# CDCgov/zoe

Measured on AMD Instinct MI355X. Metric: read-alignments/sec (150 bp vs 2 kb ref), higher is better.
Workload: dtype int16

## Files before the change

include/zoe_sw.h:

```cpp
#ifndef ZOE_SW_H
#define ZOE_SW_H

#include <stddef.h>
#include <stdint.h>

#ifdef __cplusplus
extern "C" {
#endif

typedef enum zsw_error {
    ZSW_OK = 0,
    ZSW_ERR_EMPTY_SEQUENCE = 1,
    ZSW_ERR_GAP_OPEN_OUT_OF_RANGE = 2,
    ZSW_ERR_GAP_EXTEND_OUT_OF_RANGE = 3,
    ZSW_ERR_BAD_GAP_WEIGHTS = 4,
    ZSW_ERR_INVALID_ARGUMENT = -1,
    ZSW_ERR_HIP = -2,
    ZSW_ERR_NO_DEVICE = -3,
    ZSW_ERR_UNSUPPORTED = -4,
    ZSW_ERR_NOT_CONFIGURED = -5
} zsw_error;

typedef enum zsw_status {
    ZSW_STATUS_SOME = 0,
// ... 139 lines not shown

zsw_error zsw_group_align_batch_from(zsw_group* group, const zsw_batch* reads, int from_width, int preset_bits, int invert,
                                     zsw_alignment* out_aln, uint8_t* out_status, uint8_t* out_tier, uint32_t* out_inc,
                                     uint8_t* out_op, uint64_t ciglet_cap, uint64_t* out_n_ciglets);
zsw_error zsw_group_align_3pass_batch_from(zsw_group* group, const zsw_batch* reads, int from_width, int preset_bits, int invert,
                                           zsw_alignment* out_aln, uint8_t* out_status, uint8_t* out_tier, uint32_t* out_inc,
                                           uint8_t* out_op, uint64_t ciglet_cap, uint64_t* out_n_ciglets);

zsw_error zsw_group_score_batch_from_device(zsw_group* group, const zsw_batch* shards, int from_width, int preset_bits,
                                            uint32_t* const* out_score, uint8_t* const* out_status);

zsw_error zsw_synth_reads(zsw_context* ctx, uint64_t seed, uint64_t first, uint64_t n, uint32_t len, uint8_t* out_device,
                          void* stream);
zsw_error zsw_synth_reads_ragged(zsw_context* ctx, uint64_t seed, uint64_t first, uint64_t n, uint32_t min_len,
                                 uint32_t max_len, const uint64_t* offsets_device, uint8_t* out_device, void* stream);
uint32_t zsw_synth_length(uint64_t seed, uint64_t index, uint32_t min_len, uint32_t max_len);

zsw_error zsw_selftest(zsw_context* ctx);

void zsw_synth_reference_host(uint64_t seed, uint64_t len, uint8_t* out);
void zsw_synth_reads_host(uint64_t seed, uint64_t first, uint64_t n, uint32_t len, const uint8_t* ref, uint32_t R,
                          uint8_t* out);
void zsw_synth_reads_ragged_host(uint64_t seed, uint64_t first, uint64_t n, uint32_t min_len, uint32_t max_len,
                                 const uint64_t* offsets, const uint8_t* ref, uint32_t R, uint8_t* out);

zsw_error zsw_timing_enable(zsw_context* ctx, int enable);
zsw_error zsw_timing_read(zsw_context* ctx, double* seconds, uint64_t* launches);
zsw_error zsw_timing_read_window(zsw_context* ctx, double* seconds, uint64_t* launches);

typedef enum zsw_option { ZSW_OPTION_EXACT_PRUNING = 1, ZSW_OPTION_MIN_SCORE = 2 } zsw_option;
zsw_error zsw_set_option(zsw_context* ctx, zsw_option option, int64_t value);

zsw_error zsw_min_score_counts(zsw_context* ctx, uint64_t* out );

typedef enum zsw_debug_flag {
    ZSW_DEBUG_SCORE_V1 = 1,
    ZSW_DEBUG_NO_TILES = 2,
    ZSW_DEBUG_NO_W32 = 4,
    ZSW_DEBUG_NO_WIDE = 8,
    ZSW_DEBUG_NO_SIDE_STREAMS = 16,
    ZSW_DEBUG_NO_PIPELINE = 32,
    ZSW_DEBUG_ALIGN_NO_PACKED = 64,
    ZSW_DEBUG_SCORE_PRUNE = 128,
    ZSW_DEBUG_SCORE_PRUNE_ANY_SIZE = 256,
    ZSW_DEBUG_PRUNE_STRIP = 512,
    ZSW_DEBUG_ALIGN_LONG_WARMUP = 1024,
    ZSW_DEBUG_SEED_NO_BAND = 2048,
    ZSW_DEBUG_SEED_WIDE_BAND = 4096,
    ZSW_DEBUG_NO_ROW_CHUNKS = 8192,
    ZSW_DEBUG_RANGES_EXACT_REVERSE = 16384,
    ZSW_DEBUG_ALIGN_NO_CERTIFICATE = 32768,
    ZSW_DEBUG_SEED_STRIP_FIRST_TIER = 65536,
    ZSW_DEBUG_SEED_DIAG_LANE_EVENTS = 131072,
    ZSW_DEBUG_SEED_NO_COSCHEDULE = 262144
} zsw_debug_flag;
zsw_error zsw_debug_set(zsw_context* ctx, uint32_t flags);

zsw_error zsw_debug_band_records(zsw_context* ctx, int32_t* records);

zsw_error zsw_debug_cert_records(zsw_context* ctx, int32_t* records);

zsw_error zsw_debug_strand_records(zsw_context* ctx, int32_t* records);

typedef enum zsw_launch_kind {
    ZSW_LAUNCH_V1_FAST = 0,
    ZSW_LAUNCH_V1_BIASED = 1,
    ZSW_LAUNCH_V2 = 2,
    ZSW_LAUNCH_WIDE = 3,
    ZSW_LAUNCH_V1_FAST_REV = 4,
    ZSW_LAUNCH_V1_BIASED_REV = 5,
    ZSW_LAUNCH_WIDE_REV = 6,
    ZSW_LAUNCH_TILE_V2 = 7,
    ZSW_LAUNCH_TILE_WIDE = 8,
    ZSW_LAUNCH_TILE_W32 = 9,
    ZSW_LAUNCH_EXACT32 = 10,
    ZSW_LAUNCH_EXACT32_WORKLIST = 11,
    ZSW_LAUNCH_SEED_WINDOW = 12,
    ZSW_LAUNCH_SEED_BAND = 13,
    ZSW_LAUNCH_PRUNED = 14,
    ZSW_LAUNCH_ROW_CHUNKS = 15
} zsw_launch_kind;
zsw_error zsw_debug_score_launches(zsw_context* ctx, uint32_t* records, uint32_t capacity, uint32_t* out_n);

zsw_error zsw_prune_rescored(zsw_context* ctx, uint64_t* out_reads);

#ifdef __cplusplus
}
#endif
#endif
```

zoe_amd/_lib.py:

```python
from __future__ import annotations

import ctypes as C
import os

_HERE = os.path.dirname(os.path.abspath(__file__))
LIB_PATH = os.path.join(_HERE, "libzoe_sw_hip.so")

ZSW_OK = 0
ERROR_NAMES = {
    0: "ZSW_OK",
    1: "ProfileError::EmptySequence",
    2: "ProfileError::GapOpenOutOfRange",
    3: "ProfileError::GapExtendOutOfRange",
    4: "ProfileError::BadGapWeights",
    -1: "ZSW_ERR_INVALID_ARGUMENT",
    -2: "ZSW_ERR_HIP",
    -3: "ZSW_ERR_NO_DEVICE",
    -4: "ZSW_ERR_UNSUPPORTED",
    -5: "ZSW_ERR_NOT_CONFIGURED",
}
MEM_HOST, MEM_DEVICE = 0, 1
DEBUG_SCORE_V1, DEBUG_NO_TILES, DEBUG_NO_W32, DEBUG_NO_WIDE, DEBUG_NO_SIDE_STREAMS, DEBUG_NO_PIPELINE, DEBUG_ALIGN_NO_PACKED = 1, 2, 4, 8, 16, 32, 64
DEBUG_SCORE_PRUNE, DEBUG_SCORE_PRUNE_ANY_SIZE, DEBUG_PRUNE_STRIP, DEBUG_ALIGN_LONG_WARMUP, DEBUG_SEED_NO_BAND, DEBUG_SEED_WIDE_BAND = 128, 256, 512, 1024, 2048, 4096
DEBUG_NO_ROW_CHUNKS = 8192
DEBUG_RANGES_EXACT_REVERSE = 16384
DEBUG_ALIGN_NO_CERTIFICATE = 32768
DEBUG_SEED_STRIP_FIRST_TIER = 65536
DEBUG_SEED_DIAG_LANE_EVENTS = 131072
DEBUG_SEED_NO_COSCHEDULE = 262144
(LAUNCH_V1_FAST, LAUNCH_V1_BIASED, LAUNCH_V2, LAUNCH_WIDE, LAUNCH_V1_FAST_REV, LAUNCH_V1_BIASED_REV, LAUNCH_WIDE_REV, LAUNCH_TILE_V2, LAUNCH_TILE_WIDE,
 LAUNCH_TILE_W32, LAUNCH_EXACT32, LAUNCH_EXACT32_WORKLIST, LAUNCH_SEED_WINDOW, LAUNCH_SEED_BAND, LAUNCH_PRUNED, LAUNCH_ROW_CHUNKS) = range(16)
OPTION_EXACT_PRUNING = 1
OPTION_MIN_SCORE = 2
INT_TYPES = {"i8": 0, "i16": 1, "i32": 2, "u8": 3, "u16": 4, "u32": 5}

SYMBOLS = [
    "zsw_pack4_host", "zsw_create", "zsw_destroy", "zsw_last_error_string", "zsw_device_count", "zsw_set_scoring", "zsw_set_reference",
    "zsw_score_batch", "zsw_score_batch_from", "zsw_score_ends_batch", "zsw_score_ranges_batch", "zsw_score_ranges_batch_from", "zsw_align_batch", "zsw_align_batch_from", "zsw_align_3pass_batch", "zsw_align_3pass_batch_from", "zsw_sneaky_snake_batch",
    "zsw_set_profile_sequence", "zsw_score_shared_batch", "zsw_score_shared_batch_from", "zsw_score_ends_shared_batch", "zsw_score_ranges_shared_batch",
    "zsw_score_ranges_shared_batch_from", "zsw_align_shared_batch", "zsw_align_shared_batch_from", "zsw_align_3pass_shared_batch", "zsw_align_3pass_shared_batch_from",
    "zsw_synth_reads", "zsw_synth_reads_ragged", "zsw_synth_length", "zsw_synth_reference_host", "zsw_synth_reads_host",
    "zsw_synth_reads_ragged_host", "zsw_selftest", "zsw_timing_enable", "zsw_timing_read", "zsw_timing_read_window", "zsw_debug_set", "zsw_debug_band_records", "zsw_debug_cert_records", "zsw_prune_rescored", "zsw_set_option",
    "zsw_group_create", "zsw_group_destroy", "zsw_group_size", "zsw_group_context", "zsw_group_last_error_string", "zsw_group_set_scoring",
    "zsw_group_set_reference", "zsw_group_score_batch_from", "zsw_group_score_batch_from_device", "zsw_group_align_batch_from",
    "zsw_group_align_3pass_batch_from",
    "zsw_set_complement", "zsw_score_strands_batch_from", "zsw_orient_batch", "zsw_align_3pass_strands_batch_from", "zsw_strand_counts", "zsw_debug_strand_records", "zsw_debug_score_launches",
    "zsw_min_score_counts",
]


class ZswBatch(C.Structure):
    _fields_ = [
        ("bases", C.c_void_p),
        ("offsets", C.c_void_p),
        ("fixed_len", C.c_uint32),
        ("n_reads", C.c_uint64),
        ("mem", C.c_int),
        ("encoding", C.c_int),
    ]


class ZswAlignment(C.Structure):
    _fields_ = [
        ("score", C.c_uint32),
        ("ref_start", C.c_uint32),
        ("ref_end", C.c_uint32),
        ("query_start", C.c_uint32),
        ("query_end", C.c_uint32),
        ("ref_len", C.c_uint32),
        ("query_len", C.c_uint32),
        ("n_ciglets", C.c_uint32),
        ("ciglet_offset", C.c_uint64),
    ]


class ZswError(RuntimeError):
    def __init__(self, code: int, detail: str = ""):
        self.code = code
        name = ERROR_NAMES.get(code, str(code))
        super().__init__(f"{name}{': ' + detail if detail else ''}")


# ... 85 lines not shown
```

zoe_amd/build.py:

```python
from __future__ import annotations

import os
import shutil
import subprocess
import sys

HERE = os.path.dirname(os.path.abspath(__file__))
CSRC = os.path.join(HERE, "csrc")
LIB = os.path.join(HERE, "libzoe_sw_hip.so")
SOURCES = ["zsw_capi.hip", "zsw_capi_shared.hip", "zsw_shared.hip", "zsw_score.hip", "zsw_align.hip", "zsw_align_pk8.hip", "zsw_align_pk16.hip", "zsw_align_pk32.hip", "zsw_align_pk64.hip", "zsw_group.hip", "zsw_threepass.hip", "zsw_filter.hip", "zsw_score_wide.hip", "zsw_score_w32.hip", "zsw_score_prune.hip", "zsw_score_seed.hip", "zsw_score_seed_m0.hip", "zsw_score_seed_m1.hip", "zsw_score_seed_m2.hip", "zsw_score_band.hip", "zsw_multi.hip", "zsw_strand.hip"]
HEADERS = ["zsw_internal.hpp", "zsw_align_dev.hpp", "zsw_align_pk.hpp", "zsw_align_pk_kernel.hpp", "zsw_score_v1.hpp", "zsw_score_v2.hpp", "zsw_handback.hpp", "zsw_score_prune.hpp", "zsw_seed.hpp", "zsw_seed_diag.hpp", "zsw_seed_diag_body.inc", "zsw_cert.hpp", "zsw_context.hpp", "zsw_shared.hpp", "zsw_score_seed.hpp", "zsw_score_seed_kernel.hpp", "zsw_align.hpp", "zsw_timer.hpp", "zsw_strand.hpp", "zsw_synth.h", "zsw_exports.map", os.path.join("..", "..", "include", "zoe_sw.h")]
ARCH = "gfx950"
EXTRA_FLAGS = {}


def _hipcc() -> str:
    for cand in (shutil.which("hipcc"), "/opt/rocm/bin/hipcc"):
        if cand and os.path.exists(cand):
            return cand
    raise RuntimeError("hipcc not found: the HIP extension cannot be built")


def needs_build() -> bool:
    if not os.path.exists(LIB):
        return True
    t = os.path.getmtime(LIB)
    deps = [os.path.join(CSRC, s) for s in SOURCES + HEADERS] + [os.path.abspath(__file__)]
    return any(os.path.exists(d) and os.path.getmtime(d) > t for d in deps)


def build(force: bool = False, verbose: bool = False) -> str:
    if not force and not needs_build():
        return LIB
    objs = []
    procs = []
    for s in SOURCES:
        src = os.path.join(CSRC, s)
        if not os.path.exists(src):
            continue
        obj = os.path.join(CSRC, s.replace(".hip", ".o"))
        cmd = [_hipcc(), f"--offload-arch={ARCH}", "-O3", "-std=c++17", "-fPIC", "-c", src, "-o", obj,
               "-Wall", "-Wno-unused-function", "-Wno-unused-result"] + EXTRA_FLAGS.get(s, [])
        if verbose:
            cmd.append("-Rpass-analysis=kernel-resource-usage")
        procs.append((s, subprocess.Popen(cmd, stdout=subprocess.PIPE, stderr=subprocess.STDOUT, text=True)))
        objs.append(obj)
    failed = False
    for s, p in procs:
        out, _ = p.communicate()
        if p.returncode != 0:
            failed = True
            sys.stderr.write(f"--- hipcc failed for {s}\n{out}\n")
        elif verbose or out.strip():
            sys.stderr.write(out)
    if failed:
        raise RuntimeError("hipcc compilation failed")
    cmd = [_hipcc(), f"--offload-arch={ARCH}", "-shared", "-fPIC", "-o", LIB, "-Wl,--version-script=" + os.path.join(CSRC, "zsw_exports.map")] + objs
    subprocess.run(cmd, check=True)
    return LIB


def fatbin_sha256(path: str = LIB) -> str:
    import hashlib
    import struct
# ... 36 lines not shown
```

zoe_amd/csrc/zsw_score.hip:

```cpp
#include <stdlib.h>

#include <algorithm>

#include "zsw_internal.hpp"
#include "zsw_score_v1.hpp"
#include "zsw_score_prune.hpp"
#include "zsw_score_seed.hpp"
#include "zsw_score_v2.hpp"
#include "zsw_handback.hpp"
#include "zsw_timer.hpp"

namespace zsw {

__global__ __launch_bounds__(64) void exact32_kernel(BatchDev b, const uint32_t* list, const uint32_t* list_count,
                                                     const uint8_t* ref, uint32_t ref_len, const ScoringDev* sc,
                                                     ResultRule rule, ScoreOut out, int32_t* scratch, uint32_t slots,
                                                     uint32_t scratch_len, const uint32_t* rev_ref_end,
                                                     const uint32_t* rev_query_end) {
    __shared__ uint8_t lut[256];
    __shared__ int32_t w[MAX_S * MAX_S];
    for (int i = threadIdx.x; i < 256; i += 64) lut[i] = sc->index_map[i];
    for (int i = threadIdx.x; i < MAX_S * MAX_S; i += 64) w[i] = sc->w[i];
    __syncthreads();
    const int S = sc->S;
// ... 507 lines not shown
        note_launch(launches, ZSW_LAUNCH_EXACT32, 0, 0, std::min(mode, 2));
        hipLaunchKernelGGL(exact32_kernel, dim3(exact_grid), dim3(64), 0, stream, bb, (const uint32_t*)nullptr,
                           (const uint32_t*)nullptr, d_ref, ref_len, d_sc, rule, out, ws.scratch, (uint32_t)ws.slots, ws.scratch_len, (const uint32_t*)nullptr, (const uint32_t*)nullptr);
        return hipGetLastError();
    };
    bool gtab_built = false;
    auto seed_items = [&](const BatchDev& bb, int g, int c, uint32_t longest, size_t work_off, uint32_t list_off, uint32_t* counter,
                          uint32_t band_grid_cap) -> hipError_t {
        if (!use_v2 || !ws.seed || !ws.seed_work || !ws.prune_fail_list || !(ws.debug & ZSW_DEBUG_SCORE_PRUNE) || (ws.debug & ZSW_DEBUG_PRUNE_STRIP))
            return hipErrorNotSupported;
        if (bb.n_items < SEED_MIN_READS && !(ws.debug & ZSW_DEBUG_SCORE_PRUNE_ANY_SIZE)) return hipErrorNotSupported;
        if (g == 32 || work_off + seed_workspace_bytes(bb.n_items, longest, band_grid_cap) > ws.seed_bytes) return hipErrorNotSupported;
        ScoreArgsV2 ap = a2;
        if (!build_tables_v2(h_sc, g, &ap) || !seed_applicable(*ws.seed, longest, ref_len, ap.limit)) return hipErrorNotSupported;
        if (!ws.seed_gtab) return hipErrorNotSupported;
        hipError_t pe = hipSuccess;
        ScoreArgsV2 ab = a2;
        const bool band_ok = !(ws.debug & ZSW_DEBUG_SEED_NO_BAND) && doubled_tables(h_sc, &ab);
        uint2* const gtab_band = ws.seed_gtab + (ref_len + 2 * SEED_GTAB_PAD);
        if (!gtab_built) {
            pe = seed_build_gtab(ap, ws.seed_gtab, stream);
            if (pe != hipSuccess) return pe;
            if (band_ok) {
                pe = seed_build_gtab(ab, gtab_band, stream);
                if (pe != hipSuccess) return pe;
            }
            gtab_built = true;
        }
        pe = hipMemsetAsync(counter, 0, 4, stream);
        if (pe != hipSuccess) return pe;
        ap.b = bb;
        int maxw = 0;
        for (int i = 0; i < h_sc.S * h_sc.S; ++i) maxw = std::max(maxw, (int)h_sc.w[i]);
        const uint64_t overlap = h_sc.gap_extend > 0 ? (uint64_t)longest + (uint64_t)longest * (uint64_t)maxw / (uint64_t)h_sc.gap_extend + 2 : ~0ull;
        const uint64_t rows = std::max<uint64_t>(4 * overlap, 2048);
        const bool row_chunks = ws.chunk_keys && !(ws.debug & ZSW_DEBUG_NO_ROW_CHUNKS) && h_sc.gap_extend > 0 && rows * 2 <= ref_len && longest < (1u << CHUNK_COL_BITS) &&
                                ref_len < (1u << CHUNK_ROW_BITS) - 2;
        const uint32_t min_thr = (ws.min_score && ws.min_counts && !out.skip_handed_back) ? min_threshold(rule, ws.min_score) : 0u;
        CoscheduleCase co{};
        co.mode = mode;
        co.G = g;
        co.mins = min_thr != 0;
        co.row_chunks = row_chunks;
        co.skip_handed_back = out.skip_handed_back;
        co.disabled = (ws.debug & ZSW_DEBUG_SEED_NO_COSCHEDULE) != 0;
        uint32_t* const n0 = counter + 32;
        static_assert(2 + NCLS <= 32, "the n0 words sit 32 behind their counters");
        bool coscheduled = false;
        pe = launch_score_seeded(ap, g, c, longest, *ws.seed, ws.seed_work + work_off, seed_workspace_bytes(bb.n_items, longest, band_grid_cap), ws.seed_gtab,
                                 ws.prune_fail_list + list_off, counter, mode, band_ok ? &ab : nullptr, gtab_band, ws.band_dbg,
                                 (ws.debug & ZSW_DEBUG_SEED_WIDE_BAND) ? 0xffffffffu : (ws.debug & ZSW_DEBUG_SCORE_PRUNE_ANY_SIZE) ? 0u : SEED_NARROW_MIN_READS, band_grid_cap, stream,
                                 ws.window_timer, out.narrow_only, out.reads_reversed && out.skip_handed_back, launches,
                                 (ws.debug & ZSW_DEBUG_SEED_STRIP_FIRST_TIER) != 0, (ws.debug & ZSW_DEBUG_SEED_DIAG_LANE_EVENTS) != 0,
                                 min_thr, ws.min_counts, &co, n0, &coscheduled);
        if (pe != hipSuccess) return pe;
        ap.b.items = ws.prune_fail_list + list_off;
        ap.n_items_dev = counter;
        ap.first_item_dev = coscheduled ? n0 : nullptr;
        if (!out.skip_handed_back) {
            if (row_chunks) {
                ap.chunk_rows = (uint32_t)rows;
                ap.chunk_overlap = (uint32_t)overlap;
                ap.chunk_keys = ws.chunk_keys;
                const uint32_t zgrid = (bb.n_items + 255) / 256;
                hipLaunchKernelGGL(chunk_zero_kernel, dim3(zgrid), dim3(256), 0, stream, ap.b.items, counter, bb.n_items, ws.chunk_keys);
                note_launch(launches, ZSW_LAUNCH_ROW_CHUNKS, (int)ap.chunk_rows, (int)ap.chunk_overlap, (int)((ref_len + ap.chunk_rows - 1) / ap.chunk_rows));
                note_launch(launches, ZSW_LAUNCH_V2, g, c, std::min(mode, 2));
                pe = launch_table_cfg_v2(ap, g, c, mode, stream);
                if (pe != hipSuccess) return pe;
                hipLaunchKernelGGL(chunk_finalize_kernel, dim3(zgrid), dim3(256), 0, stream, ap.b, counter, ws.chunk_keys, ap.limit, rule, out, std::min(mode, 2));
                pe = hipGetLastError();
            } else {
                HandbackLaunch plan[HANDBACK_MAX_LAUNCHES];
                ScoreArgsV2 tabs[HANDBACK_MAX_LAUNCHES];
                int n_tabs = 0;
                const int n_plan = handback_plan(kCfgs, N_CFGS, longest, g, c, bb.n_items, [&](int g2) {
                    tabs[n_tabs] = a2;
                    if (!build_tables_v2(h_sc, g2, &tabs[n_tabs])) return false;
                    ++n_tabs;
                    return true;
                }, plan);
                for (int k = 0, t = 0; k < n_plan && pe == hipSuccess; ++k) {
                    ScoreArgsV2 ah = ap;
                    if (plan[k].own_tables) {
                        ah = tabs[t++];
                        ah.b = ap.b;
                        ah.n_items_dev = counter;
                        ah.first_item_dev = ap.first_item_dev;
                    }
                    ah.b.n_items = plan[k].grid_items;
                    ah.gate_lo = plan[k].lo;
                    ah.gate_hi = plan[k].hi;
                    note_launch(launches, ZSW_LAUNCH_V2, plan[k].G, plan[k].C, std::min(mode, 2));
                    pe = launch_table_cfg_v2(ah, plan[k].G, plan[k].C, mode, stream);
                }
            }
        }
        if (pe != hipSuccess) return pe;
        if (!out.skip_handed_back) hipLaunchKernelGGL(add_count_kernel, dim3(1), dim3(1), 0, stream, counter, ws.prune_fail_count + 1);
        return hipGetLastError();
    };
    auto prune_items = [&](const BatchDev& bb, int cls, uint32_t n_cls) -> hipError_t {
        if (!(use_v2 || wide) || !ws.prune_work || !(ws.debug & ZSW_DEBUG_SCORE_PRUNE)) return hipErrorNotSupported;
        if (!wide && !(ws.debug & ZSW_DEBUG_PRUNE_STRIP)) return hipErrorNotSupported;
        if (bb.n_items < PR_MIN_READS && !(ws.debug & ZSW_DEBUG_SCORE_PRUNE_ANY_SIZE)) return hipErrorNotSupported;
        const int last = n_cls < bb.n_items ? cls + 1 : cls;
        ScoreArgsV2 ap = a2;
// ... 318 lines not shown
```

zoe_amd/csrc/zsw_score_seed.hip:

```cpp
#include <hipcub/hipcub.hpp>

#include <algorithm>
#include <vector>

#include "zsw_score_seed.hpp"
#include "zsw_score_v2.hpp"
#include "zsw_timer.hpp"

namespace zsw {

namespace {

struct SeedArgs {
    BatchDev b;
    const ScoringDev* sc;
    SeedParams sp;
    const uint2* table;
    uint32_t first, n;
    uint32_t* keys;
    uint32_t* ids;
    uint32_t* info;
    uint32_t* masks;
    uint32_t* band_masks;
    uint8_t* band_dfb;
    uint32_t* codes;
    uint32_t cs;
    uint32_t key_bias, fail_key;
    uint32_t ref_len;
    uint32_t* fail_list;
    uint32_t* fail_count;
    bool reversed;
    uint32_t min_thr;
    ScoreOut out;
    uint32_t* min_count;
};

constexpr uint32_t SEED_STAGE_LEN = 160;

template <bool STAGED, bool MINS>
__global__ __launch_bounds__(256) void seed_kernel(SeedArgs a) {
    __shared__ uint16_t cell_lut[256];
    __shared__ __attribute__((aligned(16))) uint8_t sbytes[STAGED ? 256 * SEED_STAGE_LEN + 16 : 16];
    {
        const int res = (int)a.sc->index_map[threadIdx.x];
        const uint32_t cellv = seed_cell(a.sp, res);
        cell_lut[threadIdx.x] = (uint16_t)((cellv & 0xffu) | (((cellv >> 8) == 0xffu ? 0xfu : ((cellv >> 8) & 3u)) << 8) | ((uint32_t)(res & 15) << 12));
    }
    const uint32_t k = blockIdx.x * 256 + threadIdx.x;
    const bool valid = k < a.n;
    uint32_t id = 0, len = 0;
    uint64_t off = 0;
    if (valid) {
        id = a.b.items ? a.b.items[a.first + k] : a.first + k;
        off = a.b.offsets ? a.b.offsets[id] : (uint64_t)id * a.b.fixed_len;
        len = a.b.offsets ? (uint32_t)(a.b.offsets[id + 1] - off) : a.b.fixed_len;
    }
    if (STAGED) {
        const uint32_t L = a.b.fixed_len;
        const uint64_t b0 = (uint64_t)(a.first + blockIdx.x * 256u) * L;
        const uint32_t cnt = min(256u, a.n - blockIdx.x * 256u) * L;
        const uint8_t* src = a.b.bases + b0;
        const uint32_t head = (uint32_t)((16u - (uint32_t)(reinterpret_cast<uintptr_t>(src) & 15u)) & 15u);
        const uint32_t shift = (16u - head) & 15u;
        for (uint32_t i = threadIdx.x; i < min(head, cnt); i += 256) sbytes[shift + i] = src[i];
        const uint32_t n16 = cnt > head ? (cnt - head) / 16 : 0;
        for (uint32_t i = threadIdx.x; i < n16; i += 256)
            *reinterpret_cast<uint4*>(&sbytes[shift + head + 16 * i]) = *reinterpret_cast<const uint4*>(src + head + 16 * i);
        for (uint32_t i = head + 16 * n16 + threadIdx.x; i < cnt; i += 256) sbytes[shift + i] = src[i];
        __syncthreads();
        off = (uint64_t)shift + (uint64_t)threadIdx.x * L;
    } else {
        __syncthreads();
    }
    SeedRead sr;
    sr.ok = 0;
    sr.t_all = sr.d_fa = sr.d_bl = 0;
    sr.bl_mask = 0;
    if (valid && len >= SEED_MIN_LEN && len < SEED_KEY_BIAS) {
        const uint8_t* bases = STAGED ? sbytes + off : a.b.bases + off;
        const bool rev = a.reversed;
        const uint2* table = a.table;
        uint32_t* code_out = a.codes ? a.codes + (size_t)k * a.cs : nullptr;
        uint32_t acc = 0;
        sr = seed_read<MINS>(
            a.sp, (int)len,
            [&](int c) {
                const uint32_t v = cell_lut[bases[rev ? (int)len - 1 - c : c]];
                if (code_out) {
                    acc |= (v >> 12) << (4 * (c & 7));
                    if ((c & 7) == 7) {
                        code_out[c >> 3] = acc;
                        acc = 0;
                    }
                }
                return (v & 0xffu) | (((v >> 8) & 0xfu) == 0xfu ? 0xff00u : (v & 0x300u));
            },
            [&](uint32_t code, uint32_t* f1, uint32_t* l1) {
                const uint2 e = table[code];
                *f1 = e.x;
                *l1 = e.y;
            });
    }
    bool below = false;
    if (MINS && valid && len > 0 && len < SEED_KEY_BIAS) {
        int bound = sr.u_whole;
        if (len < SEED_MIN_LEN) {
            const uint8_t* bases = STAGED ? sbytes + off : a.b.bases + off;
            bound = 0;
            for (uint32_t c = 0; c < len; ++c) bound += (int)(cell_lut[bases[c]] & 0xffu);
        }
        below = seed_below_min(bound, a.min_thr);
        if (below) {
            a.out.score[id] = 0;
            a.out.status[id] = ZSW_STATUS_BELOW_MIN_SCORE;
            if (a.out.tier) a.out.tier[id] = 0;
            if (a.out.ref_end) a.out.ref_end[id] = 0;
            if (a.out.query_end) a.out.query_end[id] = 0;
        }
    }
    if (MINS) {
        const unsigned long long mb = __ballot(below);
        if (mb && (threadIdx.x & 63) == 0) atomicAdd(a.min_count, (uint32_t)__popcll(mb));
    }
    const bool fail = valid && !sr.ok && !below;
    if (valid) {
        a.keys[k] = (sr.ok && !below) ? (uint32_t)(sr.dt + (int)a.key_bias) : a.fail_key;
        a.ids[k] = k;
        a.info[k] = (uint32_t)sr.t_all | ((uint32_t)sr.d_fa << 16) | ((uint32_t)sr.d_bl << 24);
        a.masks[k] = sr.bl_mask;
        if (a.codes) {
            a.band_masks[k] = sr.fa_mask | (sr.fb_mask << 16);
            a.band_dfb[k] = (uint8_t)sr.d_fb;
            uint32_t* code_row = a.codes + (size_t)k * a.cs;
            const bool swept = len >= SEED_MIN_LEN && len < SEED_KEY_BIAS;
            const uint32_t full = swept ? len >> 3 : 0;
            if (full < a.cs) {
                uint32_t tail = 0xffffffffu;
                if (swept && (len & 7u)) {
                    const uint8_t* bases = STAGED ? sbytes + off : a.b.bases + off;
                    tail = 0;
                    for (uint32_t c = full * 8; c < full * 8 + 8; ++c)
                        tail |= (c < len ? (uint32_t)(cell_lut[bases[a.reversed ? len - 1 - c : c]] >> 12) : 15u) << (4 * (c & 7));
                }
                code_row[full] = tail;
                for (uint32_t d = full + 1; d < a.cs; ++d) code_row[d] = 0xffffffffu;
            }
        }
    }
    const unsigned long long m = __ballot(fail);
    if (m) {
        const int lane = threadIdx.x & 63;
        const int leader = __ffsll((long long)m) - 1;
        uint32_t base = 0;
        if (lane == leader) base = atomicAdd(a.fail_count, (uint32_t)__popcll(m));
        base = (uint32_t)__shfl((int)base, leader, 64);
        if (fail) a.fail_list[base + (uint32_t)__popcll(m & ((1ull << lane) - 1ull))] = id;
    }
}

__global__ void seed_gtab_kernel(const uint8_t* ref, uint32_t ref_len, const ScoringDev* sc, ScoreArgsV2 a, uint2* gtab) {
    const uint32_t i = blockIdx.x * blockDim.x + threadIdx.x;
    if (i >= ref_len + 2 * SEED_GTAB_PAD) return;
    const int row = (int)i - SEED_GTAB_PAD;
    const int idx = (row >= 0 && row < (int)ref_len) ? (int)sc->index_map[ref[row]] : NEUTRAL;
    gtab[i] = make_uint2(a.wtab[idx][0], a.wtab[idx][1]);
}

size_t round256(size_t x) { return (x + 255) & ~(size_t)255; }

size_t sort_temp_bytes(uint32_t n) {
    size_t bytes = 0, sel = 0;
    (void)hipcub::DeviceRadixSort::SortPairs(nullptr, bytes, (const uint32_t*)nullptr, (uint32_t*)nullptr, (const uint32_t*)nullptr,
                                             (uint32_t*)nullptr, (int)n, 0, 32, (hipStream_t)0);
    (void)hipcub::DeviceSelect::Flagged(nullptr, sel, (const uint32_t*)nullptr, (const uint8_t*)nullptr, (uint32_t*)nullptr, (uint32_t*)nullptr,
                                        (int)n, (hipStream_t)0);
    return std::max(bytes, sel);
}

}

uint32_t seed_codes_stride(uint32_t max_len) { return (max_len + 7) / 8 + 1; }

size_t seed_workspace_bytes(uint32_t n, uint32_t max_len, uint32_t band_grid_cap) {
    SeedParams p{};
    p.M1 = SEED_M1;
    p.M1_per8 = SEED_M1_PER8;
    p.Wd = SEED_WD;
    p.Wd_per16 = SEED_WD_PER16;
    return 7 * round256((size_t)n * 4 + 8) + round256((size_t)n + 8) + round256((size_t)n * seed_codes_stride(max_len) * 4 + 8) +
           round256(sort_temp_bytes(n)) + round256(seed_band_buffer_bytes(p, n, max_len, band_grid_cap)) + 256;
}

bool seed_applicable(const SeedIndex& ix, uint32_t max_len, uint32_t ref_len, uint32_t limit) {
    if (!ix.valid || !ix.usable || !ix.d_table || ref_len == 0 || ref_len >= (1u << 24)) return false;
    if (max_len < SEED_MIN_LEN || max_len > SEED_MAX_LEN) return false;
    return (uint64_t)ix.params.maxw * max_len + 8 < limit;
}

hipError_t launch_score_seeded(const ScoreArgsV2& a2, int G, int C, uint32_t max_len, const SeedIndex& ix, uint8_t* work, size_t work_bytes,
                               uint2* gtab, uint32_t* fail_list, uint32_t* fail_count, int mode, const ScoreArgsV2* band_tabs, const uint2* gtab_band, int32_t* band_dbg,
                               uint32_t narrow_min_reads, uint32_t band_grid_cap, hipStream_t stream, KernelTimer* window_timer, bool narrow_only, bool reads_reversed,
                               std::vector<uint32_t>* launches, bool strip_first_tier, bool diag_lane_events, uint32_t min_thr, uint32_t* min_counts,
                               const CoscheduleCase* co, uint32_t* n0, bool* coscheduled) {
    const uint32_t n = a2.b.n_items;
    if (coscheduled) *coscheduled = false;
    if (!min_counts) min_thr = 0;
    if (n == 0) return hipSuccess;
    if (!work || !gtab || work_bytes < seed_workspace_bytes(n, max_len, band_grid_cap)) return hipErrorNotSupported;
    const bool band = band_tabs != nullptr && gtab_band != nullptr && seed_band_applicable(ix.params, max_len, band_tabs->K, band_tabs->limit);
    const size_t per = round256((size_t)n * 4 + 8);
    uint32_t* keys = reinterpret_cast<uint32_t*>(work);
    uint32_t* keys_out = reinterpret_cast<uint32_t*>(work + per);
    uint32_t* ids = reinterpret_cast<uint32_t*>(work + 2 * per);
    uint32_t* order = reinterpret_cast<uint32_t*>(work + 3 * per);
    uint32_t* info = reinterpret_cast<uint32_t*>(work + 4 * per);
    uint32_t* masks = reinterpret_cast<uint32_t*>(work + 5 * per);
    uint32_t* band_masks = reinterpret_cast<uint32_t*>(work + 6 * per);
    uint8_t* p8 = work + 7 * per;
    uint8_t* band_dfb = p8;
    p8 += round256((size_t)n + 8);
    const uint32_t cs = seed_codes_stride(max_len);
    uint32_t* codes = reinterpret_cast<uint32_t*>(p8);
    p8 += round256((size_t)n * cs * 4 + 8);
    void* temp = p8;
    p8 += round256(sort_temp_bytes(n));
    uint2* band_buf = reinterpret_cast<uint2*>(p8);
    size_t temp_bytes = sort_temp_bytes(n);
    int key_bits = 1;
    while ((1ull << key_bits) < (uint64_t)a2.ref_len + 2ull * SEED_KEY_BIAS + 2 && key_bits < 32) ++key_bits;
    const uint32_t fail_key = key_bits >= 32 ? 0xffffffffu : (1u << key_bits) - 1u;

    SeedArgs s;
    s.b = a2.b;
    s.sc = a2.sc;
    s.sp = ix.params;
    s.table = reinterpret_cast<const uint2*>(ix.d_table);
    s.first = 0;
    s.n = n;
    s.keys = keys;
    s.ids = ids;
    s.info = info;
    s.masks = masks;
    s.band_masks = band_masks;
    s.band_dfb = band_dfb;
    s.codes = band ? codes : nullptr;
    s.cs = cs;
    s.key_bias = SEED_KEY_BIAS;
    s.fail_key = fail_key;
    s.ref_len = a2.ref_len;
    s.fail_list = fail_list;
    s.fail_count = fail_count;
    s.reversed = reads_reversed;
    s.min_thr = min_thr;
    s.out = a2.out;
    s.min_count = min_counts;
    const bool staged = !s.b.offsets && !s.b.items && s.b.fixed_len <= SEED_STAGE_LEN;
    if (min_thr) {
        if (staged) hipLaunchKernelGGL((seed_kernel<true, true>), dim3((n + 255) / 256), dim3(256), 0, stream, s);
        else hipLaunchKernelGGL((seed_kernel<false, true>), dim3((n + 255) / 256), dim3(256), 0, stream, s);
    } else if (staged)
        hipLaunchKernelGGL((seed_kernel<true, false>), dim3((n + 255) / 256), dim3(256), 0, stream, s);
    else
        hipLaunchKernelGGL((seed_kernel<false, false>), dim3((n + 255) / 256), dim3(256), 0, stream, s);
    hipError_t e = hipcub::DeviceRadixSort::SortPairs(temp, temp_bytes, (const uint32_t*)keys, keys_out, (const uint32_t*)ids, order, (int)n, 0,
                                                      key_bits, stream);
    if (e != hipSuccess) return e;

    if (band) {
        SeedBandArgs b;
        b.b = a2.b;
        b.ref_len = a2.ref_len;
        b.ge2 = band_tabs->ge2;
        b.gd2 = band_tabs->gd2;
        b.floor0 = band_tabs->floor0;
        b.rule = a2.rule;
        b.out = a2.out;
        b.sp = ix.params;
        b.n = n;
        b.order = order;
        b.keys = keys;
        b.info = info;
        b.band_masks = band_masks;
        b.band_dfb = band_dfb;
        b.codes = codes;
        b.cs = cs;
        b.gtab = gtab_band;
        b.bnd = band_buf;
        b.dbg = band_dbg;
        b.nb = seed_band_rows(ix.params, max_len);
        b.grid = seed_band_grid(n, band_grid_cap);
        b.key_bias = SEED_KEY_BIAS;
        b.fail_key = fail_key;
        b.fail_list = fail_list;
        b.fail_count = fail_count;
        b.wu0 = ix.params.M1;
        b.wu_per16 = 2 * ix.params.M1_per8;
        b.wd0 = ix.params.Wd;
        b.wd_per32 = 2 * ix.params.Wd_per16;
        b.n_dev = nullptr;
        b.retry = nullptr;
        b.min_thr = min_thr;
        b.min_count = min_counts ? min_counts + 1 : nullptr;
        uint32_t* queue1 = reinterpret_cast<uint32_t*>(work + 3 * per + (size_t)n * 4) + 1;
        uint32_t* queue2 = reinterpret_cast<uint32_t*>(work + (size_t)n * 4);
        e = hipMemsetAsync(queue1, 0, 4, stream);
        if (e != hipSuccess) return e;
        e = hipMemsetAsync(queue2, 0, 8, stream);
        if (e != hipSuccess) return e;
        uint32_t* accepted = queue2 + 1;
        b.next_pair = queue2;
        if (window_timer) window_timer->begin(stream);
        if (max_len <= SEED_NARROW_MAX_LEN && n >= narrow_min_reads) {
            uint8_t* retry = reinterpret_cast<uint8_t*>(ids);
// ... 146 lines not shown
```

zoe_amd/csrc/zsw_score_seed.hpp:

```cpp
#pragma once
#include "zsw_handback.hpp"
#include "zsw_internal.hpp"
#include "zsw_seed.hpp"

namespace zsw {

constexpr int SEED_M1 = 24;
constexpr int SEED_M1_PER8 = 1;
constexpr int SEED_M2 = 16;
constexpr int SEED_DN = 4;
constexpr int SEED_TOL = 8;
constexpr int SEED_DM = 4;
constexpr int SEED_WD = 9;
constexpr int SEED_WD_PER16 = 1;
constexpr int SEED_NARROW_WU = 8, SEED_NARROW_WU_PER16 = 0, SEED_NARROW_WD = 6, SEED_NARROW_WD_PER32 = 0;
constexpr uint32_t SEED_BAIL_RATIO = 40;
constexpr uint32_t SEED_BAIL_BELOW = 16384;
constexpr int SEED_SECOND_WU = 16, SEED_SECOND_WU_PER16 = 1, SEED_SECOND_WD = 8, SEED_SECOND_WD_PER32 = 1;
constexpr uint32_t SEED_NARROW_MAX_LEN = 640;
constexpr uint32_t SEED_NARROW_MIN_READS = 200000;
constexpr int SEED_BAND_SLACK = 32;
constexpr int SEED_DIAG_SLACK = 1;
constexpr uint32_t SEED_DIAG_MAX_LEN = 255;
constexpr uint32_t SEED_BAND_MAX_GRID = 1024;
// ... 41 lines not shown
    ResultRule rule;
    ScoreOut out;
    SeedParams sp;
    uint32_t n;
    const uint32_t* order;
    const uint32_t* keys;
    const uint32_t* info;
    const uint32_t* band_masks;
    const uint8_t* band_dfb;
    const uint32_t* codes;
    uint32_t cs;
    const uint2* gtab;
    uint2* bnd;
    uint32_t nb;
    uint32_t grid;
    int wu0, wu_per16, wd0, wd_per32;
    const uint32_t* n_dev;
    uint32_t* next_pair;
    uint8_t* retry;
    uint32_t* accepted = nullptr;
    bool bail_check = false;
    uint32_t bail_below = 0;
    bool diag_lane_events = false;
    int* dbg;
    uint32_t key_bias, fail_key;
    uint32_t* fail_list;
    uint32_t* fail_count;
    uint32_t min_thr = 0;
    uint32_t* min_count = nullptr;
};
uint32_t seed_band_rows(const SeedParams& p, uint32_t max_len);
uint32_t seed_band_grid(uint32_t n, uint32_t grid_cap);
size_t seed_band_buffer_bytes(const SeedParams& p, uint32_t n, uint32_t max_len, uint32_t grid_cap);
bool seed_band_applicable(const SeedParams& p, uint32_t max_len, uint32_t rebase_rows, uint32_t limit);
hipError_t launch_seed_band(const SeedBandArgs& a, int mode, bool narrow_strips, hipStream_t stream, bool diagonal = false);
bool seed_diag_applicable(uint32_t max_len, uint32_t rebase_rows);

struct ScoreArgsV2;
hipError_t launch_seed_diag_handback(const SeedBandArgs& a, const ScoreArgsV2& hb, int G, int C, hipStream_t stream);

constexpr uint32_t SEED_BAND_CLASS_MIN_GRID = 64;
inline uint32_t seed_band_class_cap(uint32_t n_class, uint32_t n_total) {
    return SEED_BAND_CLASS_MIN_GRID + (uint32_t)((uint64_t)SEED_BAND_MAX_GRID * n_class / (n_total ? n_total : 1));
}
size_t seed_workspace_bytes(uint32_t n, uint32_t max_len, uint32_t band_grid_cap = SEED_BAND_MAX_GRID);
bool seed_applicable(const SeedIndex& ix, uint32_t max_len, uint32_t ref_len, uint32_t limit);
hipError_t seed_build_gtab(const ScoreArgsV2& a2, uint2* gtab, hipStream_t stream);
hipError_t launch_score_seeded(const ScoreArgsV2& a2, int G, int C, uint32_t max_len, const SeedIndex& ix, uint8_t* work, size_t work_bytes,
                               uint2* gtab, uint32_t* fail_list, uint32_t* fail_count, int mode, const ScoreArgsV2* band_tabs, const uint2* gtab_band, int32_t* band_dbg,
                               uint32_t narrow_min_reads, uint32_t band_grid_cap, hipStream_t stream, KernelTimer* window_timer, bool narrow_only = false, bool reads_reversed = false,
                               std::vector<uint32_t>* launches = nullptr , bool strip_first_tier = false ,
                               bool diag_lane_events = false ,
                               uint32_t min_thr = 0 , uint32_t* min_counts = nullptr ,
                               const CoscheduleCase* co = nullptr, uint32_t* n0 = nullptr, bool* coscheduled = nullptr);
hipError_t seed_index_update(SeedIndex* ix, const ScoringDev& sc, const uint8_t* h_ref, size_t ref_len);
void seed_index_release(SeedIndex* ix);

hipError_t launch_seed_window_m0(const SeedWindowArgs& a, int G, int C, hipStream_t stream);
hipError_t launch_seed_window_m1(const SeedWindowArgs& a, int G, int C, hipStream_t stream);
hipError_t launch_seed_window_m2(const SeedWindowArgs& a, int G, int C, hipStream_t stream);

}
```

Before: 690.8 million.

## Add packed-nibble seed kernel staging fixed-length reads in LDS

Adds a seed_packed_kernel for fixed-length staged batches. It cooperatively packs each read's bases into 4-bit residue codes in LDS using 8-byte window loads and a shared LUT, writes the code rows as it goes, then runs the seed voting from the packed rows with branch-light unrolled span-bound and vote helpers. The code-row emission moves out of seed_emit so both kernels share the emit path. This is meant to cut the per-thread byte-wise global loads and LUT lookups of the old seed kernel, at the cost of dynamic LDS use and a separate code path that has to produce identical results. A debug flag restores the old kernel.

```diff
diff --git a/include/zoe_sw.h b/include/zoe_sw.h
--- a/include/zoe_sw.h
+++ b/include/zoe_sw.h
@@ -215,7 +215,8 @@
     ZSW_DEBUG_ALIGN_NO_CERTIFICATE = 32768,
     ZSW_DEBUG_SEED_STRIP_FIRST_TIER = 65536,
     ZSW_DEBUG_SEED_DIAG_LANE_EVENTS = 131072,
-    ZSW_DEBUG_SEED_NO_COSCHEDULE = 262144
+    ZSW_DEBUG_SEED_NO_COSCHEDULE = 262144,
+    ZSW_DEBUG_SEED_PLAIN_KERNEL = 524288
 } zsw_debug_flag;
 zsw_error zsw_debug_set(zsw_context* ctx, uint32_t flags);
 
diff --git a/zoe_amd/_lib.py b/zoe_amd/_lib.py
--- a/zoe_amd/_lib.py
+++ b/zoe_amd/_lib.py
@@ -28,6 +28,7 @@
 DEBUG_SEED_STRIP_FIRST_TIER = 65536
 DEBUG_SEED_DIAG_LANE_EVENTS = 131072
 DEBUG_SEED_NO_COSCHEDULE = 262144
+DEBUG_SEED_PLAIN_KERNEL = 524288
 (LAUNCH_V1_FAST, LAUNCH_V1_BIASED, LAUNCH_V2, LAUNCH_WIDE, LAUNCH_V1_FAST_REV, LAUNCH_V1_BIASED_REV, LAUNCH_WIDE_REV, LAUNCH_TILE_V2, LAUNCH_TILE_WIDE,
  LAUNCH_TILE_W32, LAUNCH_EXACT32, LAUNCH_EXACT32_WORKLIST, LAUNCH_SEED_WINDOW, LAUNCH_SEED_BAND, LAUNCH_PRUNED, LAUNCH_ROW_CHUNKS) = range(16)
 OPTION_EXACT_PRUNING = 1
diff --git a/zoe_amd/build.py b/zoe_amd/build.py
--- a/zoe_amd/build.py
+++ b/zoe_amd/build.py
@@ -9,7 +9,7 @@
 CSRC = os.path.join(HERE, "csrc")
 LIB = os.path.join(HERE, "libzoe_sw_hip.so")
 SOURCES = ["zsw_capi.hip", "zsw_capi_shared.hip", "zsw_shared.hip", "zsw_score.hip", "zsw_align.hip", "zsw_align_pk8.hip", "zsw_align_pk16.hip", "zsw_align_pk32.hip", "zsw_align_pk64.hip", "zsw_group.hip", "zsw_threepass.hip", "zsw_filter.hip", "zsw_score_wide.hip", "zsw_score_w32.hip", "zsw_score_prune.hip", "zsw_score_seed.hip", "zsw_score_seed_m0.hip", "zsw_score_seed_m1.hip", "zsw_score_seed_m2.hip", "zsw_score_band.hip", "zsw_multi.hip", "zsw_strand.hip"]
-HEADERS = ["zsw_internal.hpp", "zsw_align_dev.hpp", "zsw_align_pk.hpp", "zsw_align_pk_kernel.hpp", "zsw_score_v1.hpp", "zsw_score_v2.hpp", "zsw_handback.hpp", "zsw_score_prune.hpp", "zsw_seed.hpp", "zsw_seed_diag.hpp", "zsw_seed_diag_body.inc", "zsw_cert.hpp", "zsw_context.hpp", "zsw_shared.hpp", "zsw_score_seed.hpp", "zsw_score_seed_kernel.hpp", "zsw_align.hpp", "zsw_timer.hpp", "zsw_strand.hpp", "zsw_synth.h", "zsw_exports.map", os.path.join("..", "..", "include", "zoe_sw.h")]
+HEADERS = ["zsw_internal.hpp", "zsw_align_dev.hpp", "zsw_align_pk.hpp", "zsw_align_pk_kernel.hpp", "zsw_score_v1.hpp", "zsw_score_v2.hpp", "zsw_handback.hpp", "zsw_score_prune.hpp", "zsw_seed.hpp", "zsw_seed_packed.hpp", "zsw_seed_diag.hpp", "zsw_seed_diag_body.inc", "zsw_cert.hpp", "zsw_context.hpp", "zsw_shared.hpp", "zsw_score_seed.hpp", "zsw_score_seed_kernel.hpp", "zsw_align.hpp", "zsw_timer.hpp", "zsw_strand.hpp", "zsw_synth.h", "zsw_exports.map", os.path.join("..", "..", "include", "zoe_sw.h")]
 ARCH = "gfx950"
 EXTRA_FLAGS = {}
 
diff --git a/zoe_amd/csrc/zsw_score.hip b/zoe_amd/csrc/zsw_score.hip
--- a/zoe_amd/csrc/zsw_score.hip
+++ b/zoe_amd/csrc/zsw_score.hip
@@ -583,7 +583,7 @@
                                  (ws.debug & ZSW_DEBUG_SEED_WIDE_BAND) ? 0xffffffffu : (ws.debug & ZSW_DEBUG_SCORE_PRUNE_ANY_SIZE) ? 0u : SEED_NARROW_MIN_READS, band_grid_cap, stream,
                                  ws.window_timer, out.narrow_only, out.reads_reversed && out.skip_handed_back, launches,
                                  (ws.debug & ZSW_DEBUG_SEED_STRIP_FIRST_TIER) != 0, (ws.debug & ZSW_DEBUG_SEED_DIAG_LANE_EVENTS) != 0,
-                                 min_thr, ws.min_counts, &co, n0, &coscheduled);
+                                 min_thr, ws.min_counts, &co, n0, &coscheduled, (ws.debug & ZSW_DEBUG_SEED_PLAIN_KERNEL) != 0);
         if (pe != hipSuccess) return pe;
         ap.b.items = ws.prune_fail_list + list_off;
         ap.n_items_dev = counter;
diff --git a/zoe_amd/csrc/zsw_score_seed.hip b/zoe_amd/csrc/zsw_score_seed.hip
--- a/zoe_amd/csrc/zsw_score_seed.hip
+++ b/zoe_amd/csrc/zsw_score_seed.hip
@@ -4,6 +4,7 @@
 #include <vector>
 
 #include "zsw_score_seed.hpp"
+#include "zsw_seed_packed.hpp"
 #include "zsw_score_v2.hpp"
 #include "zsw_timer.hpp"
 
@@ -36,6 +37,10 @@
 };
 
 constexpr uint32_t SEED_STAGE_LEN = 160;
+static_assert(SEED_STAGE_LEN == (uint32_t)SEED_PACKED_MAX_LEN, "the staged batches are the ones seed_packed_kernel takes");
+
+template <bool MINS>
+__device__ __forceinline__ void seed_emit(const SeedArgs& a, uint32_t k, uint32_t id, uint32_t len, bool valid, const SeedRead& sr, int bound);
 
 template <bool STAGED, bool MINS>
 __global__ __launch_bounds__(256) void seed_kernel(SeedArgs a) {
@@ -76,6 +81,8 @@
     sr.ok = 0;
     sr.t_all = sr.d_fa = sr.d_bl = 0;
     sr.bl_mask = 0;
+    sr.dt = sr.d_fb = sr.u_whole = 0;
+    sr.fa_mask = sr.fb_mask = 0;
     if (valid && len >= SEED_MIN_LEN && len < SEED_KEY_BIAS) {
         const uint8_t* bases = STAGED ? sbytes + off : a.b.bases + off;
         const bool rev = a.reversed;
@@ -101,14 +108,35 @@
                 *l1 = e.y;
             });
     }
+    int bound = sr.u_whole;
+    if (MINS && valid && len > 0 && len < SEED_MIN_LEN) {
+        const uint8_t* bases = STAGED ? sbytes + off : a.b.bases + off;
+        bound = 0;
+        for (uint32_t c = 0; c < len; ++c) bound += (int)(cell_lut[bases[c]] & 0xffu);
+    }
+    seed_emit<MINS>(a, k, id, len, valid, sr, bound);
+    if (valid && a.codes) {
+        uint32_t* code_row = a.codes + (size_t)k * a.cs;
+        const bool swept = len >= SEED_MIN_LEN && len < SEED_KEY_BIAS;
+        const uint32_t full = swept ? len >> 3 : 0;
+        if (full < a.cs) {
+            uint32_t tail = 0xffffffffu;
+            if (swept && (len & 7u)) {
+                const uint8_t* bases = STAGED ? sbytes + off : a.b.bases + off;
+                tail = 0;
+                for (uint32_t c = full * 8; c < full * 8 + 8; ++c)
+                    tail |= (c < len ? (uint32_t)(cell_lut[bases[a.reversed ? len - 1 - c : c]] >> 12) : 15u) << (4 * (c & 7));
+            }
+            code_row[full] = tail;
+            for (uint32_t d = full + 1; d < a.cs; ++d) code_row[d] = 0xffffffffu;
+        }
+    }
+}
+
+template <bool MINS>
+__device__ __forceinline__ void seed_emit(const SeedArgs& a, uint32_t k, uint32_t id, uint32_t len, bool valid, const SeedRead& sr, int bound) {
     bool below = false;
     if (MINS && valid && len > 0 && len < SEED_KEY_BIAS) {
-        int bound = sr.u_whole;
-        if (len < SEED_MIN_LEN) {
-            const uint8_t* bases = STAGED ? sbytes + off : a.b.bases + off;
-            bound = 0;
-            for (uint32_t c = 0; c < len; ++c) bound += (int)(cell_lut[bases[c]] & 0xffu);
-        }
         below = seed_below_min(bound, a.min_thr);
         if (below) {
             a.out.score[id] = 0;
@@ -131,20 +159,6 @@
         if (a.codes) {
             a.band_masks[k] = sr.fa_mask | (sr.fb_mask << 16);
             a.band_dfb[k] = (uint8_t)sr.d_fb;
-            uint32_t* code_row = a.codes + (size_t)k * a.cs;
-            const bool swept = len >= SEED_MIN_LEN && len < SEED_KEY_BIAS;
-            const uint32_t full = swept ? len >> 3 : 0;
-            if (full < a.cs) {
-                uint32_t tail = 0xffffffffu;
-                if (swept && (len & 7u)) {
-                    const uint8_t* bases = STAGED ? sbytes + off : a.b.bases + off;
-                    tail = 0;
-                    for (uint32_t c = full * 8; c < full * 8 + 8; ++c)
-                        tail |= (c < len ? (uint32_t)(cell_lut[bases[a.reversed ? len - 1 - c : c]] >> 12) : 15u) << (4 * (c & 7));
-                }
-                code_row[full] = tail;
-                for (uint32_t d = full + 1; d < a.cs; ++d) code_row[d] = 0xffffffffu;
-            }
         }
     }
     const unsigned long long m = __ballot(fail);
@@ -158,6 +172,71 @@
     }
 }
 
+constexpr uint32_t SEED_PACKED_LUT_WORDS = 64 + 8;
+size_t seed_packed_lds_bytes(uint32_t L) { return 4 * (size_t)(SEED_PACKED_LUT_WORDS + 256u * (uint32_t)seed_packed_res_words((int)L)); }
+
+template <bool MINS>
+__global__ __launch_bounds__(256) void seed_packed_kernel(SeedArgs a) {
+    extern __shared__ uint32_t seed_lds[];
+    const uint32_t t = threadIdx.x;
+    const uint32_t L = a.b.fixed_len;
+    const uint32_t res_words = (uint32_t)seed_packed_res_words((int)L);
+    uint8_t* entry_lut = reinterpret_cast<uint8_t*>(seed_lds);
+    uint16_t* cell16 = reinterpret_cast<uint16_t*>(seed_lds + 64);
+    uint32_t* res_rows = seed_lds + SEED_PACKED_LUT_WORDS;
+    entry_lut[t] = a.sc->index_map[t];
+    if (t < 16) cell16[t] = (uint16_t)seed_cell(a.sp, (int)t);
+    __syncthreads();
+    const uint32_t r0 = blockIdx.x * 256u;
+    const uint32_t nr = min(256u, a.n - r0);
+    const uint8_t* src = a.b.bases + (uint64_t)(a.first + r0) * L;
+    const int cnt = (int)(nr * L);
+    const uint32_t rw = (L + 7) / 8;
+    const uint32_t cs = a.cs;
+    const bool swept = L >= SEED_MIN_LEN;
+    const bool rev = a.reversed;
+    const uint32_t magic = seed_div_magic((int)cs);
+    uint32_t* codes_out = a.codes ? a.codes + (size_t)r0 * cs : nullptr;
+    for (uint32_t i = t; i < nr * cs; i += 256) {
+        const uint32_t r = (uint32_t)seed_div((int)i, magic), d = i - r * cs;
+        uint32_t res = 0xffffffffu;
+        if (d < rw) {
+            const int ncols = min(8, (int)L - 8 * (int)d);
+            const uint64_t w = seed_pack_window(src, cnt, (int)L, (int)r, (int)d, rev);
+            res = seed_pack8(w, ncols, [&](uint32_t byte) { return (uint32_t)entry_lut[byte]; });
+            res_rows[r * res_words + d] = res;
+        }
+        if (codes_out) codes_out[i] = swept ? res : 0xffffffffu;
+    }
+    __syncthreads();
+    const uint32_t k = r0 + t;
+    const bool valid = t < nr;
+    const uint32_t id = a.first + k;
+    const uint32_t* res_row = res_rows + t * res_words;
+    SeedRead sr;
+    sr.ok = 0;
+    sr.t_all = sr.d_fa = sr.d_bl = 0;
+    sr.bl_mask = 0;
+    sr.dt = sr.d_fb = sr.u_whole = 0;
+    sr.fa_mask = sr.fb_mask = 0;
+    if (valid && swept) {
+        const uint2* table = a.table;
+        sr = seed_read_packed<MINS>(
+            a.sp, (int)L, res_row, [&](uint32_t res) { return (uint32_t)cell16[res]; },
+            [&](uint32_t code, uint32_t* f1, uint32_t* l1) {
+                const uint2 e = table[code];
+                *f1 = e.x;
+                *l1 = e.y;
+            });
+    }
+    int bound = sr.u_whole;
+    if (MINS && valid && L > 0 && !swept) {
+        bound = 0;
+        for (uint32_t c = 0; c < L; ++c) bound += (int)(cell16[(res_row[c >> 3] >> (4 * (c & 7))) & 15u] & 0xffu);
+    }
+    seed_emit<MINS>(a, k, id, L, valid, sr, bound);
+}
+
 __global__ void seed_gtab_kernel(const uint8_t* ref, uint32_t ref_len, const ScoringDev* sc, ScoreArgsV2 a, uint2* gtab) {
     const uint32_t i = blockIdx.x * blockDim.x + threadIdx.x;
     if (i >= ref_len + 2 * SEED_GTAB_PAD) return;
@@ -201,7 +280,7 @@
                                uint2* gtab, uint32_t* fail_list, uint32_t* fail_count, int mode, const ScoreArgsV2* band_tabs, const uint2* gtab_band, int32_t* band_dbg,
                                uint32_t narrow_min_reads, uint32_t band_grid_cap, hipStream_t stream, KernelTimer* window_timer, bool narrow_only, bool reads_reversed,
                                std::vector<uint32_t>* launches, bool strip_first_tier, bool diag_lane_events, uint32_t min_thr, uint32_t* min_counts,
-                               const CoscheduleCase* co, uint32_t* n0, bool* coscheduled) {
+                               const CoscheduleCase* co, uint32_t* n0, bool* coscheduled, bool plain_seed_kernel) {
     const uint32_t n = a2.b.n_items;
     if (coscheduled) *coscheduled = false;
     if (!min_counts) min_thr = 0;
@@ -255,10 +334,14 @@
     s.out = a2.out;
     s.min_count = min_counts;
     const bool staged = !s.b.offsets && !s.b.items && s.b.fixed_len <= SEED_STAGE_LEN;
+    const bool packed = staged && !plain_seed_kernel && cs <= (uint32_t)SEED_PACKED_RES_WORDS_MAX;
     if (min_thr) {
-        if (staged) hipLaunchKernelGGL((seed_kernel<true, true>), dim3((n + 255) / 256), dim3(256), 0, stream, s);
+        if (packed) hipLaunchKernelGGL((seed_packed_kernel<true>), dim3((n + 255) / 256), dim3(256), seed_packed_lds_bytes(s.b.fixed_len), stream, s);
+        else if (staged) hipLaunchKernelGGL((seed_kernel<true, true>), dim3((n + 255) / 256), dim3(256), 0, stream, s);
         else hipLaunchKernelGGL((seed_kernel<false, true>), dim3((n + 255) / 256), dim3(256), 0, stream, s);
-    } else if (staged)
+    } else if (packed)
+        hipLaunchKernelGGL((seed_packed_kernel<false>), dim3((n + 255) / 256), dim3(256), seed_packed_lds_bytes(s.b.fixed_len), stream, s);
+    else if (staged)
         hipLaunchKernelGGL((seed_kernel<true, false>), dim3((n + 255) / 256), dim3(256), 0, stream, s);
     else
         hipLaunchKernelGGL((seed_kernel<false, false>), dim3((n + 255) / 256), dim3(256), 0, stream, s);
diff --git a/zoe_amd/csrc/zsw_score_seed.hpp b/zoe_amd/csrc/zsw_score_seed.hpp
--- a/zoe_amd/csrc/zsw_score_seed.hpp
+++ b/zoe_amd/csrc/zsw_score_seed.hpp
@@ -117,7 +117,8 @@
                                std::vector<uint32_t>* launches = nullptr , bool strip_first_tier = false ,
                                bool diag_lane_events = false ,
                                uint32_t min_thr = 0 , uint32_t* min_counts = nullptr ,
-                               const CoscheduleCase* co = nullptr, uint32_t* n0 = nullptr, bool* coscheduled = nullptr);
+                               const CoscheduleCase* co = nullptr, uint32_t* n0 = nullptr, bool* coscheduled = nullptr,
+                               bool plain_seed_kernel = false );
 hipError_t seed_index_update(SeedIndex* ix, const ScoringDev& sc, const uint8_t* h_ref, size_t ref_len);
 void seed_index_release(SeedIndex* ix);
 
diff --git a/zoe_amd/csrc/zsw_seed_packed.hpp b/zoe_amd/csrc/zsw_seed_packed.hpp
--- /dev/null
+++ b/zoe_amd/csrc/zsw_seed_packed.hpp
@@ -0,0 +1,174 @@
+#pragma once
+#include "zsw_seed.hpp"
+
+namespace zsw {
+
+constexpr int SEED_PACKED_MAX_LEN = 160;
+ZSW_SEED_HD int seed_packed_res_words(int len) { return ((len + 7) / 8) | 1; }
+constexpr int SEED_PACKED_RES_WORDS_MAX = 21;
+
+template <class Entry>
+ZSW_SEED_HD uint32_t seed_pack8(uint64_t w, int ncols, Entry entry) {
+    const uint32_t w0 = (uint32_t)w, w1 = (uint32_t)(w >> 32);
+    uint32_t h0 = 0, h1 = 0;
+#pragma unroll
+    for (int k = 0; k < 4; ++k) {
+        h0 |= (entry((w0 >> (8 * k)) & 0xffu) & 15u) << (4 * k);
+        h1 |= (entry((w1 >> (8 * k)) & 0xffu) & 15u) << (4 * k);
+    }
+    const uint32_t live = ncols < 8 ? (1u << (4 * ncols)) - 1u : 0xffffffffu;
+    return ((h0 | (h1 << 16)) & live) | ~live;
+}
+
+ZSW_SEED_HD uint64_t seed_pack_window(const uint8_t* src, int cnt, int len, int r, int d, bool rev) {
+    const int lo = r * len + (rev ? len - 8 - 8 * d : 8 * d);
+    uint64_t w = 0;
+    if (lo >= 0 && lo + 8 <= cnt) {
+        __builtin_memcpy(&w, src + lo, 8);
+    } else {
+        for (int b = 0; b < 8; ++b)
+            if (lo + b >= 0 && lo + b < cnt) w |= (uint64_t)src[lo + b] << (8 * b);
+    }
+    return rev ? __builtin_bswap64(w) : w;
+}
+
+ZSW_SEED_HD int seed_span_bound_packed(int m, const uint32_t* pots, int t_all, uint32_t set, int lambda) {
+    int best = 0, cnt = 0;
+    int low = 0;
+#pragma unroll
+    for (int b = 0; b <= SEED_MAX_KMERS; ++b) {
+        if (b > m) continue;
+        if (b > 0) {
+            const int la = (int)(pots[b - 1] & 0xffffu) - lambda * cnt;
+            low = la < low ? la : low;
+        }
+        const int hi = b == m ? t_all : (int)(pots[b < SEED_MAX_KMERS ? b : 0] >> 16);
+        const int v = hi - lambda * cnt - low;
+        best = v > best ? v : best;
+        if (b < m && ((set >> b) & 1u)) ++cnt;
+    }
+    return best;
+}
+
+constexpr int SEED_VOTE_FAR = -(1 << 30);
+ZSW_SEED_HD int seed_vote_far(int m, uint32_t has, const int* dlo, const int* dhi, int tol, int* dt) {
+    int best = 0, bd = 0;
+    const int step = m > 8 ? 2 : 1;
+    const uint32_t span = 2u * (uint32_t)tol;
+#pragma unroll
+    for (int i = 0; i < 2 * SEED_MAX_KMERS; ++i) {
+        const int j = i >> 1;
+        if (j >= m || (j % step) != 0) continue;
+        const int d = (i & 1) ? dhi[j] : dlo[j];
+        const bool candidate = ((has >> j) & 1u) && !((i & 1) && dhi[j] == dlo[j]);
+        const int e = tol - d;
+        int sup = 0;
+#pragma unroll
+        for (int k = 0; k < SEED_MAX_KMERS; ++k) {
+            if (k >= m) continue;
+            sup += ((uint32_t)(dlo[k] + e) <= span || (uint32_t)(dhi[k] + e) <= span) ? 1 : 0;
+        }
+        if (candidate && sup > best) {
+            best = sup;
+            bd = d;
+        }
+    }
+    *dt = bd;
+    return best;
+}
+
+template <bool WHOLE = false, class Cell16, class Lookup>
+ZSW_SEED_HD SeedRead seed_read_packed(const SeedParams& p, int len, const uint32_t* res_row, Cell16 cell16, Lookup look) {
+    SeedRead out;
+    out.ok = 0;
+    out.dt = 0;
+    out.t_all = 0;
+    out.d_fa = 0;
+    out.d_bl = 0;
+    out.bl_mask = 0;
+    out.d_fb = 0;
+    out.fa_mask = out.fb_mask = 0;
+    int m, stride, c0;
+    seed_layout(len, p.K, p.spacer, &m, &stride, &c0);
+    const int lam = seed_lambda(p, stride);
+    uint32_t pots[SEED_MAX_KMERS], codes[SEED_MAX_KMERS];
+    uint32_t usable = 0;
+    int pot = 0;
+    uint32_t word = 0;
+    auto cell = [&](int c) {
+        if ((c & 7) == 0) word = res_row[c >> 3];
+        return cell16((word >> (4 * (c & 7))) & 15u);
+    };
+    int c = 0;
+#pragma unroll
+    for (int j = 0; j < SEED_MAX_KMERS; ++j) {
+        pots[j] = codes[j] = 0;
+        if (j >= m) continue;
+        const int cj = c0 + j * stride;
+        int run = p.ins_col;
+        for (; c < cj; ++c) {
+            const int wpc = (int)(cell(c) & 0xffu);
+            pot += wpc;
+            run += wpc + p.ge;
+        }
+        uint32_t code = 0, lo = 0, hi = 0;
+        bool ok = j == 0 || run >= lam;
+        for (int k = 0; k < p.K; ++k, ++c) {
+            const uint32_t x = cell(c);
+            pot += (int)(x & 0xffu);
+            ok = ok && (x >> 8) != 0xffu;
+            code |= ((x >> 8) & 3u) << (2 * k);
+            if (k == 0) lo = (uint32_t)pot;
+            if (k == p.K - 2) hi = (uint32_t)pot;
+        }
+        pots[j] = lo | (hi << 16);
+        if (ok) {
+            usable |= 1u << j;
+            codes[j] = code;
+        }
+    }
+    for (; c < len; ++c) pot += (int)(cell(c) & 0xffu);
+    uint32_t f1s[SEED_MAX_KMERS], l1s[SEED_MAX_KMERS];
+#pragma unroll
+    for (int j = 0; j < SEED_MAX_KMERS; ++j) {
+        f1s[j] = l1s[j] = 0;
+        look(codes[j], &f1s[j], &l1s[j]);
+    }
+    int dlo[SEED_MAX_KMERS], dhi[SEED_MAX_KMERS];
+    bool hasb[SEED_MAX_KMERS];
+    uint32_t has = 0;
+#pragma unroll
+    for (int j = 0; j < SEED_MAX_KMERS; ++j) {
+        const int cj = c0 + j * stride;
+        hasb[j] = ((usable >> j) & 1u) && f1s[j] != 0;
+        has |= hasb[j] ? 1u << j : 0u;
+        dlo[j] = hasb[j] ? (int)(f1s[j] - 1) - cj : SEED_VOTE_FAR;
+        dhi[j] = hasb[j] ? (int)(l1s[j] - 1) - cj : SEED_VOTE_FAR;
+    }
+    out.t_all = pot;
+    out.u_whole = pot;
+    if (m == 0) return out;
+    if (WHOLE) out.u_whole = seed_span_bound_packed(m, pots, pot, usable & ~has, lam);
+    int dt = 0;
+    const int support = seed_vote_far(m, has, dlo, dhi, p.tol, &dt);
+    if (support < (m >= 3 ? 2 : 1)) return out;
+#pragma unroll
+    for (int i = 0; i < SEED_MAX_KMERS; ++i) {
+        const int ci = c0 + i * stride;
+        const bool u = (usable >> i) & 1u;
+        out.fa_mask |= (u && (!hasb[i] || dlo[i] >= dt - p.Dn)) ? 1u << i : 0u;
+        out.bl_mask |= (u && (!hasb[i] || dhi[i] + ci < dt + len + p.M2)) ? 1u << i : 0u;
+        out.fb_mask |= (u && (!hasb[i] || dhi[i] <= dt + p.Dm)) ? 1u << i : 0u;
+    }
+    const int u_fa = seed_span_bound_packed(m, pots, pot, out.fa_mask, lam);
+    const int u_bl = seed_span_bound_packed(m, pots, pot, out.bl_mask, lam);
+    const int u_fb = seed_span_bound_packed(m, pots, pot, out.fb_mask, lam);
+    out.ok = 1;
+    out.dt = dt;
+    out.d_fa = pot - u_fa > 255 ? 255 : pot - u_fa;
+    out.d_bl = pot - u_bl > 255 ? 255 : pot - u_bl;
+    out.d_fb = pot - u_fb > 255 ? 255 : pot - u_fb;
+    return out;
+}
+
+}
```

Result: faster. 754.0 million, median of 6 (+9.1%).
